# OpenImagingLab/AdaptiveISP

Hardware: AMD Instinct MI355X
Metric: ISP+YOLO forward images/sec @1280x720 bs8 (higher is better)
Workload: dtype bf16; 1 GPU; batch 8 x 1280x720 fp32 RGB, 5-step ISP schedule ['E', 'CCM', 'NLM', 'Shr', 'T'] (teacher-forced, policy/heads evaluated every step) + YOLOv3 forward @1280x736 bf16 (random-init weights); per_gpu_batch=8, global_batch=8, parallelism=replicas x1

## Files before the change

### adaptiveisp_amd/csrc/yolo_api.hip

```cpp
#include "yolo_internal.h"
#include <algorithm>
#include <atomic>
#include <cstdlib>
#include <cstring>
#include <mutex>
#include <unordered_map>
#include <vector>

using namespace adayolo;

static void magic_div(unsigned d, unsigned* magic, int* sh) {
    if (d <= 1) { *magic = 0; *sh = -1; return; }
    int L = 0;
    while ((1ull << L) < d) ++L;
    const unsigned long long num = 1ull << (31 + L);
    *magic = (unsigned)((num + d - 1) / d);
    *sh = L - 1;
}

static int code(hipError_t e, int on_invalid = ADAYOLO_ELAUNCH) {
    if (e == hipErrorInvalidValue) return on_invalid;
    return e == hipSuccess ? ADAYOLO_OK : ADAYOLO_ELAUNCH;
}

// ... 618 lines not shown
                       void* stream) {
    if (!in || !out || B <= 0 || H <= 0 || W <= 0 || C <= 0) return ADAYOLO_EINVAL;
    if (C % 8 || in_cstride % 8 || out_cstride % 8 || in_cstride < C || out_cstride < C) return ADAYOLO_ESHAPE;
    return code(launch_upsample2x(in, in_cstride, out, out_cstride, B, H, W, C, static_cast<hipStream_t>(stream)));
}

int adayolo_detect_decode(const void* raw, int raw_cstride, float* pred, int pred_rows, int row_offset,
                          const float* anchors_px, float det_stride, int B, int ny, int nx, int na, int no,
                          void* stream) {
    if (!raw || !pred || !anchors_px || B <= 0 || ny <= 0 || nx <= 0 || na <= 0 || no < 5) return ADAYOLO_EINVAL;
    if (raw_cstride < na * no || row_offset < 0 || row_offset + na * ny * nx > pred_rows) return ADAYOLO_ESHAPE;
    return code(launch_detect_decode(raw, raw_cstride, pred, pred_rows, row_offset, anchors_px, det_stride, B, ny, nx, na,
                                     no, static_cast<hipStream_t>(stream)));
}

size_t adayolo_nms_workspace_bytes(int n) {
    const size_t nb = (size_t)((n > 0 ? n : 0) + 63) / 64;
    return (size_t)(n > 0 ? n : 0) * nb * 8 + 8;
}

int adayolo_nms(const float* boxes_xyxy, int n, float iou_thres, int max_det, void* workspace, int32_t* keep,
                int32_t* num_keep, void* stream) {
    if (n < 0 || max_det <= 0 || !keep || !num_keep || (n > 0 && (!boxes_xyxy || !workspace))) return ADAYOLO_EINVAL;
    if (n > 30000 * 4) return ADAYOLO_ESHAPE;
    if (!(iou_thres >= 0.0f && iou_thres <= 1.0f)) return ADAYOLO_EINVAL;
    return code(launch_nms(boxes_xyxy, n, iou_thres, max_det, static_cast<unsigned long long*>(workspace), keep, num_keep,
                           static_cast<hipStream_t>(stream)));
}

static int detloss_check(const adayolo_loss_args* a, bool bwd) {
// ... 27 lines not shown
```

### adaptiveisp_amd/csrc/yolo_conv_pq.hip

```cpp
#include "yolo_device.h"
#include <type_traits>
#include <cstdlib>

namespace adayolo {
namespace pq {

template <int N> using IC = std::integral_constant<int, N>;

constexpr int BN = 128, BK = 32;
constexpr int kRow = BK * 2;
template <int MI> struct Geo {
    static constexpr int BM = 64 * MI;
    static constexpr int kATile = BM * kRow;
    static constexpr int kBuf = (BM + BN) * kRow;
    static constexpr int kRing = 3 * kBuf;
    static constexpr int kEpi = 4 * 32 * MI * kEpiPitch;
    static constexpr int kSmem = kRing > kEpi ? kRing : kEpi;
    static constexpr int NA = MI;
    static constexpr int NP = MI + 2;
};

__device__ __forceinline__ void fence() { __builtin_amdgcn_sched_barrier(0); }
#define PQ_SGB(mask, n) __builtin_amdgcn_sched_group_barrier(mask, n, 0)

template <int ABL, int MI>
__global__ __launch_bounds__(256, 2) void k_conv_pq(const ConvArgs a) {
    constexpr int BM = Geo<MI>::BM, kATile = Geo<MI>::kATile, kBuf = Geo<MI>::kBuf, NA = Geo<MI>::NA, NP = Geo<MI>::NP;
    constexpr int H1 = NP / 2;
    extern __shared__ __attribute__((aligned(16))) unsigned char smem[];
    const int tid = threadIdx.x, lane = tid & 63;
    const int wave = __builtin_amdgcn_readfirstlane(tid >> 6);
    const int wm = wave >> 1, wn = wave & 1;
    const int lid = xcd_remap(blockIdx.x, a.mtiles * a.ntiles);
    const int m0 = (lid / a.ntiles) * BM, n0 = (lid % a.ntiles) * BN;
    const int Kw = a.ks * a.ks * a.Cin;
    const int nK = Kw / BK;

    const unsigned guard = 2u * (unsigned)(a.W + 1) * (unsigned)a.in_cs;
    const __amdgpu_buffer_rsrc_t rsA =
        __builtin_amdgcn_make_buffer_rsrc((void*)((const unsigned char*)a.in - guard), 0, kRecords, kDescFlags);
// ... 189 lines not shown
#pragma unroll
                for (int it = 0; it < 4; ++it) {
                    r[it] = u32x4{0u, 0u, 0u, 0u};
                    if (ok[it]) r[it] = *reinterpret_cast<const u32x4*>(rp + (4 * mi + it) * rstep);
                }
            }
#pragma unroll
            for (int ni = 0; ni < 2; ++ni)
#pragma unroll
                for (int qd = 0; qd < 4; ++qd) {
                    f32x2 x0 = {acc[ni][mi][4 * qd], acc[ni][mi][4 * qd + 1]}, x1 = {acc[ni][mi][4 * qd + 2], acc[ni][mi][4 * qd + 3]};
                    if (kSilu) { x0 = silu_pk(x0); x1 = silu_pk(x1); }
                    *reinterpret_cast<u32x2*>(wr + mi * 32 * kEpiPitch + (ni * 32 + 8 * qd) * 2) =
                        u32x2{pack_bf16x2(x0.x, x0.y), pack_bf16x2(x1.x, x1.y)};
                }
            asm volatile("s_waitcnt lgkmcnt(0)" ::: "memory");
#pragma unroll
            for (int it = 0; it < 4; ++it) v[it] = *reinterpret_cast<const u32x4*>(rd + (mi * 32 + it * 8) * kEpiPitch);
            if (kKeep) {
#pragma unroll
                for (int it = 0; it < 4; ++it) {
                    if (ok[it]) *reinterpret_cast<u32x4*>(a.pre + (long)(mrow + 8 * (4 * mi + it)) * a.pre_cs + n) = v[it];
                    if (kAct) {
#pragma unroll
                        for (int j = 0; j < 4; ++j) v[it][j] = silu_bf16x2(v[it][j]);
                    }
                }
            }
            if (kRes) {
#pragma unroll
// ... 14 lines not shown
                }
                if (a.out) {
#pragma unroll
                    for (int it = 0; it < 4; ++it)
                        if (ok[it]) __builtin_nontemporal_store(v[it], reinterpret_cast<u32x4*>(op + (4 * mi + it) * ostep));
                }
#pragma unroll
                for (int it = 0; it < 4; ++it) {
#pragma unroll
                    for (int j = 0; j < 4; ++j) v[it][j] = dsilu_bf16x2(v[it][j], p[it][j]);
                    if (ok[it])
                        __builtin_nontemporal_store(v[it], reinterpret_cast<u32x4*>(a.gpre + (long)(mrow + 8 * (4 * mi + it)) * a.gpre_cs + n));
                }
                continue;
            }
#pragma unroll
            for (int it = 0; it < 4; ++it)
                if (ok[it]) __builtin_nontemporal_store(v[it], reinterpret_cast<u32x4*>(op + (4 * mi + it) * ostep));
        }
    };
    const std::false_type no{};
    const std::true_type yes{};
    if (a.gpre) {
        if (a.res) epilogue(no, yes, no, yes); else epilogue(no, no, no, yes);
    } else if (a.pre) {
        if (a.act == ADAYOLO_ACT_SILU) { if (a.res) epilogue(yes, yes, yes, no); else epilogue(yes, no, yes, no); }
        else { if (a.res) epilogue(no, yes, yes, no); else epilogue(no, no, yes, no); }
    } else if (a.act == ADAYOLO_ACT_SILU) {
        if (a.res) epilogue(yes, yes, no, no); else epilogue(yes, no, no, no);
    } else {
        if (a.res) epilogue(no, yes, no, no); else epilogue(no, no, no, no);
    }
}

template <int ABL, int MI = 4>
static hipError_t launch(ConvArgs a, hipStream_t s) {
    constexpr int kSmem = Geo<MI>::kSmem;
    static_assert(2 * kSmem <= 160 * 1024, "two workgroups per CU");
    a.mtiles = (a.M + Geo<MI>::BM - 1) / Geo<MI>::BM;
    auto kern = k_conv_pq<ABL, MI>;
    static bool configured = false;
    if (!configured) {
        hipError_t e = hipFuncSetAttribute(reinterpret_cast<const void*>(kern),
                                           hipFuncAttributeMaxDynamicSharedMemorySize, kSmem);
        if (e != hipSuccess) return e;
        configured = true;
    }
    int smem_bytes = kSmem;
#ifdef ADAYOLO_MEASURE
    static const int extra = getenv("ADAYOLO_PQ_EXTRA_SMEM") ? atoi(getenv("ADAYOLO_PQ_EXTRA_SMEM")) : 0;
    smem_bytes += extra;
    if (extra) (void)hipFuncSetAttribute(reinterpret_cast<const void*>(kern), hipFuncAttributeMaxDynamicSharedMemorySize, smem_bytes);
#endif
    hipLaunchKernelGGL(kern, dim3(a.mtiles * a.ntiles), dim3(256), smem_bytes, s, a);
    return hipGetLastError();
}

}

hipError_t launch_conv_pq(ConvArgs a, hipStream_t s, int variant) {
    const long nK = (long)a.ks * a.ks * a.Cin / 32;
    if (a.Cin % 32 || a.Cout % 128 || nK < 3 || a.sh_hw < 0 || a.sh_w < 0 || a.d2s_c) return hipErrorInvalidValue;
    const unsigned long long lim = 0xFFFFFF00ull - 64;
    const unsigned long long in_b = 2ull * a.B * a.H * a.W * a.in_cs + 4ull * (a.W + 1) * a.in_cs + 2ull * a.Cin;
    if (in_b > lim || 2ull * a.Cout * a.ks * a.ks * a.Cin > lim) return hipErrorInvalidValue;
    a.ntiles = a.Cout / pq::BN;
#ifdef ADAYOLO_MEASURE
    if (variant == 81) return pq::launch<1>(a, s);
    if (variant == 82) return pq::launch<2>(a, s);
    if (variant == 83) return pq::launch<3>(a, s);
#endif
    if (variant == 85) return pq::launch<0, 2>(a, s);
    return pq::launch<0>(a, s);
}

}
```

### adaptiveisp_amd/csrc/yolo_device.h

```cpp
#pragma once
#include "yolo_internal.h"

namespace adayolo {

typedef __attribute__((ext_vector_type(8))) __bf16 bf16x8;
typedef __attribute__((ext_vector_type(2))) __bf16 bf16x2;
typedef __attribute__((ext_vector_type(2))) float f32x2;
typedef __attribute__((ext_vector_type(4))) float f32x4;
typedef __attribute__((ext_vector_type(16))) float f32x16;
typedef __attribute__((ext_vector_type(2))) unsigned int u32x2;
typedef __attribute__((ext_vector_type(4))) unsigned int u32x4;
typedef __attribute__((ext_vector_type(4))) short s16x4;
typedef __attribute__((address_space(3))) void* lds_ptr_t;
typedef const __attribute__((address_space(1))) void* gbl_ptr_t;

__device__ __forceinline__ float bf16_to_f32(unsigned short h) { return __uint_as_float(((unsigned)h) << 16); }
__device__ __forceinline__ float lo_f(unsigned v) { return __uint_as_float(v << 16); }
__device__ __forceinline__ float hi_f(unsigned v) { return __uint_as_float(v & 0xFFFF0000u); }
__device__ __forceinline__ unsigned pack_bf16x2(float lo, float hi) {
    return __builtin_bit_cast(unsigned, __builtin_convertvector(f32x2{lo, hi}, bf16x2));
}
__device__ __forceinline__ unsigned short f32_to_bf16(float f) {
    unsigned u = __float_as_uint(f);
    u += 0x7FFFu + ((u >> 16) & 1u);
// ... 62 lines not shown
    return x * r;
}
__device__ __forceinline__ unsigned silu_bf16x2(unsigned v) {
    const f32x2 y = silu_pk(f32x2{__uint_as_float(v << 16), __uint_as_float(v & 0xFFFF0000u)});
    return __builtin_bit_cast(unsigned, __builtin_convertvector(y, bf16x2));
}
__device__ __forceinline__ float dsilu_f32(float g, float p) {
    const float s = __builtin_amdgcn_rcpf(1.0f + __builtin_amdgcn_exp2f(-1.44269504088896341f * p));
    return g * __builtin_fmaf(p * s, 1.0f - s, s);
}
__device__ __forceinline__ unsigned dsilu_bf16x2(unsigned g, unsigned p) {
    const f32x2 y = {dsilu_f32(__uint_as_float(g << 16), __uint_as_float(p << 16)),
                     dsilu_f32(__uint_as_float(g & 0xFFFF0000u), __uint_as_float(p & 0xFFFF0000u))};
    return __builtin_bit_cast(unsigned, __builtin_convertvector(y, bf16x2));
}
template <bool SILU>
__device__ __forceinline__ void bias_act_pack4(float a0, float a1, float a2, float a3, const float4 b, unsigned& lo, unsigned& hi) {
    f32x2 x0 = f32x2{a0, a1} + f32x2{b.x, b.y};
    f32x2 x1 = f32x2{a2, a3} + f32x2{b.z, b.w};
    if (SILU) { x0 = silu_pk(x0); x1 = silu_pk(x1); }
    lo = __builtin_bit_cast(unsigned, __builtin_convertvector(x0, bf16x2));
    hi = __builtin_bit_cast(unsigned, __builtin_convertvector(x1, bf16x2));
}

}
```

### adaptiveisp_amd/csrc/yolo_internal.h

```cpp
#pragma once
#include <hip/hip_runtime.h>
#include <stdint.h>
#include "../../include/adayolo.h"

namespace adayolo {

struct ConvArgs {
    const unsigned short* in; int in_cs;
    const unsigned short* w; const float* bias;
    const unsigned short* res; int res_cs;
    unsigned short* out; int out_cs;
    int B, H, W, Cin, Cout, Ho, Wo, ks, stride, pad, act;
    int M;
    int mtiles, ntiles;
    unsigned magic_hw, magic_w;
    int sh_hw, sh_w;
    const unsigned short* w2; const float* bias2;
    unsigned short* out2; int out2_cs;
    unsigned short* pre; int pre_cs;
    float* partial = nullptr; int* tickets = nullptr; int ksplit = 1;
    unsigned short* gpre = nullptr; int gpre_cs = 0;
    int d2s_c = 0;
    int chain_tile = 0;
};

struct ChainHead { int layer, lid, flag, pad; };
struct ChainDeps {
    int in_lo, in_n_need;
    int res_lo, res_n_need;
};
struct ChainArgs {
    unsigned char* ws;
    int* host_err;
    int off_layers, off_heads, off_deps, total, ndone;
    int stagger;
};
hipError_t launch_conv_chain(const ChainArgs& c, int grid, hipStream_t s);
enum ShapeFamily { kShapePp = 0, kShapePp128 = 1 };
int mfma_shape(ShapeFamily f);
hipError_t launch_conv_dma(ConvArgs a, hipStream_t s, int variant);
hipError_t launch_conv_dma2(ConvArgs a, hipStream_t s, int variant);
hipError_t launch_conv_small(ConvArgs a, hipStream_t s, int variant);
hipError_t launch_conv_pp(ConvArgs a, hipStream_t s, int variant);
hipError_t launch_conv_pp128(ConvArgs a, hipStream_t s, int variant);
size_t conv_pp128_splitk_bytes(const ConvArgs& a, int S);
hipError_t launch_conv_pp128_splitk(ConvArgs a, hipStream_t s, int S, void* workspace, size_t workspace_bytes);
hipError_t launch_bottleneck256(const void* x, int x_cs, const void* w1, const float* b1, const void* w2, const float* b2,
                                void* out, int out_cs, int B, int H, int W, hipStream_t s);
hipError_t launch_bottleneck_ws(const void* x, int x_cs, const void* w1, const float* b1, const void* w2, const float* b2,
                                void* out, int out_cs, int B, int H, int W, int C, hipStream_t s);
hipError_t launch_conv_k1(ConvArgs a, hipStream_t s);
hipError_t launch_conv_pq(ConvArgs a, hipStream_t s, int variant);
hipError_t launch_conv_ws(ConvArgs a, hipStream_t s, int variant);
hipError_t launch_stem(const float* img, const float* w, const float* bias, void* out, int out_cs, int B, int H,
                       int W, int Hp, int pad_top, float pad_value, int act, hipStream_t s, void* pre = nullptr, int pre_cs = 0);
hipError_t launch_letterbox_pack(const float* img, void* out, int out_cs, int B, int H, int W, int Hp, int pad_top,
                                 float pad_value, hipStream_t s);
hipError_t launch_stem_down(const float* img, const float* w0, const float* b0, const void* w1, const float* b1, void* out,
                            int out_cs, int B, int H, int W, int Hp, int pad_top, float pad_value, const void* w2,
                            const float* b2, void* out2, int out2_cs, hipStream_t s);
hipError_t launch_upsample2x(const void* in, int in_cs, void* out, int out_cs, int B, int H, int W, int C,
                             hipStream_t s);
hipError_t launch_detect_decode(const void* raw, int raw_cs, float* pred, int pred_rows, int row_offset,
                                const float* anchors_px, float det_stride, int B, int ny, int nx, int na, int no,
                                hipStream_t s);
hipError_t launch_silu_fwd(const void* pre, int pre_cs, const void* res, int res_cs, void* out, int out_cs, long npix,
                           int C, hipStream_t s);
// ... 15 lines not shown
```

### adaptiveisp_amd/csrc/yolo_misc.hip

```cpp
#include "yolo_device.h"

namespace adayolo {

constexpr int S_TW = 64, S_TH = 16, S_LW = S_TW + 2, S_LH = S_TH + 2;

__global__ __launch_bounds__(256) void k_stem(const float* __restrict__ img, const float* __restrict__ w,
                                              const float* __restrict__ bias, unsigned short* __restrict__ out,
                                              int out_cs, int H, int W, int Hp, int pad_top, float pad_value, int act,
                                              unsigned short* __restrict__ pre, int pre_cs) {
    __shared__ float tile[3 * S_LH * S_LW];
    const int tid = threadIdx.x, lane = tid & 63, wave = tid >> 6;
    const int b = blockIdx.z, x0 = blockIdx.x * S_TW, y0 = blockIdx.y * S_TH;
    const long plane = (long)H * W;
    const float* src = img + (long)b * 3 * plane;
    for (int i = tid; i < 3 * S_LH * S_LW; i += 256) {
        const int c = i / (S_LH * S_LW), r = i - c * (S_LH * S_LW);
        const int ly = r / S_LW, lx = r - ly * S_LW;
        const int gy = y0 - 1 + ly, gx = x0 - 1 + lx;
        float v = 0.0f;
        if (gy >= 0 && gy < Hp && gx >= 0 && gx < W) {
            const int sy = gy - pad_top;
            v = (sy >= 0 && sy < H) ? src[c * plane + (long)sy * W + gx] : pad_value;
        }
        tile[i] = v;
// ... 119 lines not shown
}

__global__ __launch_bounds__(256) void k_detect_decode(const unsigned short* __restrict__ raw, int raw_cs,
                                                       float* __restrict__ pred, int pred_rows, int row_offset,
                                                       const float* __restrict__ anchors_px, float det_stride, int ny,
                                                       int nx, int na, int no) {
    const int an = blockIdx.y;
    const long b = blockIdx.z;
    const int per_map = ny * nx * no;
    const float aw = anchors_px[2 * an], ah = anchors_px[2 * an + 1];
    const unsigned short* src = raw + b * ny * nx * raw_cs + an * no;
    float* dst = pred + (b * pred_rows + row_offset + (long)an * ny * nx) * no;
    for (int i = blockIdx.x * 256 + threadIdx.x; i < per_map; i += gridDim.x * 256) {
        const int cell = i / no, j = i - cell * no;
        const float t = bf16_to_f32(src[(long)cell * raw_cs + j]);
        const float s = __builtin_amdgcn_rcpf(1.0f + __builtin_amdgcn_exp2f(-1.44269504088896341f * t));
        float v = s;
        if (j < 4) {
            const int y = cell / nx, x = cell - y * nx;
            const float s2 = s * 2.0f;
            v = (j == 0) ? (s2 + ((float)x - 0.5f)) * det_stride
              : (j == 1) ? (s2 + ((float)y - 0.5f)) * det_stride
              : (j == 2) ? s2 * s2 * aw : s2 * s2 * ah;
        }
        dst[i] = v;
    }
}

constexpr int DC = 32;
__global__ __launch_bounds__(256) void k_detect_decode_tiled(const unsigned short* __restrict__ raw, int raw_cs,
                                                             float* __restrict__ pred, int pred_rows, int row_offset,
                                                             const float* __restrict__ anchors_px, float det_stride,
                                                             int ny, int nx, int na, int no) {
    extern __shared__ __attribute__((aligned(16))) unsigned char dsm[];
    unsigned short* l16 = reinterpret_cast<unsigned short*>(dsm);
    const int ncell = ny * nx;
    const int cell0 = blockIdx.x * DC;
    const int nc = min(DC, ncell - cell0);
// ... 24 lines not shown
                ++j;
                const int wr = j == no;
                j = wr ? 0 : j; an += wr;
            }
        }
    }
    __syncthreads();
    float* boxf = reinterpret_cast<float*>(dsm + (size_t)na * DC * no * 2);
    for (int idx = threadIdx.x; idx < na * nc; idx += 256) {
        const int an = (int)(((float)idx + 0.5f) / (float)nc), cl = idx - an * nc;
        const int cell = cell0 + cl;
        const int y = (int)(((float)cell + 0.5f) * inv_nx), x = cell - y * nx;
        const unsigned short* lp = l16 + (an * DC + cl) * no;
        float sg[4];
#pragma unroll
        for (int u = 0; u < 4; ++u) sg[u] = __builtin_amdgcn_rcpf(1.0f + __builtin_amdgcn_exp2f(-1.44269504088896341f * bf16_to_f32(lp[u])));
        float* bo = boxf + (an * DC + cl) * 4;
        bo[0] = (sg[0] * 2.0f + ((float)x - 0.5f)) * det_stride;
        bo[1] = (sg[1] * 2.0f + ((float)y - 0.5f)) * det_stride;
        bo[2] = (sg[2] * 2.0f) * (sg[2] * 2.0f) * anchors_px[2 * an];
        bo[3] = (sg[3] * 2.0f) * (sg[3] * 2.0f) * anchors_px[2 * an + 1];
    }
    __syncthreads();
    const int total = nc * no;
    for (int an = 0; an < na; ++an) {
        float* dst = pred + (b * pred_rows + row_offset + (long)an * ncell + cell0) * no;
        const unsigned char* la = dsm + (long)an * DC * no * 2;
        for (int e4 = threadIdx.x; 4 * e4 < total; e4 += 256) {
            const uint2 p = *reinterpret_cast<const uint2*>(la + 8 * e4);
            const float t[4] = {__uint_as_float(p.x << 16), __uint_as_float(p.x & 0xFFFF0000u),
                                __uint_as_float(p.y << 16), __uint_as_float(p.y & 0xFFFF0000u)};
            f32x4 o;
#pragma unroll
            for (int u = 0; u < 4; ++u) o[u] = __builtin_amdgcn_rcpf(1.0f + __builtin_amdgcn_exp2f(-1.44269504088896341f * t[u]));
            const int cl = (int)(((float)(4 * e4) + 0.5f) * inv_no), j0 = 4 * e4 - cl * no;
            if (j0 < 4 || j0 + 3 >= no) {
#pragma unroll
                for (int u = 0; u < 4; ++u) {
                    const int wrp = j0 + u >= no;
                    const int j = j0 + u - (wrp ? no : 0);
                    if (j < 4) o[u] = boxf[(an * DC + cl + wrp) * 4 + j];
                }
            }
            __builtin_nontemporal_store(o, reinterpret_cast<f32x4*>(dst + 4 * e4));
        }
    }
}

hipError_t launch_detect_decode(const void* raw, int raw_cs, float* pred, int pred_rows, int row_offset,
// ... 25 lines not shown
```

### adaptiveisp_amd/yolo/_lib.py

```python
import ctypes
import os

import torch

_HERE = os.path.dirname(os.path.dirname(os.path.abspath(__file__)))
LIB_PATH = os.environ.get("ADAYOLO_LIB") or os.path.join(_HERE, "csrc", "libadayolo.so")
ABI_VERSION = 9
ACT_NONE, ACT_SILU = 0, 1
EXPORTS = ("adayolo_conv_fwd", "adayolo_conv_fwd_variant", "adayolo_conv_fused1x1_fwd", "adayolo_conv1x1_stream_fwd", "adayolo_bottleneck256_fwd", "adayolo_bottleneck_ws_fwd", "adayolo_conv_keep_fwd", "adayolo_conv_splitk_fwd", "adayolo_conv_dsilu_fwd", "adayolo_conv_s2grad_fwd", "adayolo_conv_splitk_workspace_bytes", "adayolo_conv_chain_workspace_bytes", "adayolo_conv_chain_prepare", "adayolo_conv_chain_fwd", "adayolo_conv_chain_status", "adayolo_conv_chain_poll", "adayolo_conv_chain_tables", "adayolo_stem_fwd", "adayolo_upsample2x", "adayolo_detect_decode", "adayolo_nms", "adayolo_nms_workspace_bytes", "adayolo_stem_fwd_act", "adayolo_stem_keep_fwd", "adayolo_stem_down_fwd", "adayolo_letterbox_pack", "adayolo_silu_fwd", "adayolo_silu_bwd",
           "adayolo_zero_insert2x", "adayolo_upsample2x_bwd", "adayolo_image_grad", "adayolo_detloss_fwd", "adayolo_detloss_bwd",
           "adayolo_strerror", "adayolo_set_mfma_shape", "adayolo_get_mfma_shape",
           "adayolo_abi_version")
_lib = None


class AdayoloError(RuntimeError):
    pass


class LossLayer(ctypes.Structure):
    _fields_ = [("raw", ctypes.c_void_p), ("cs", ctypes.c_int), ("ny", ctypes.c_int), ("nx", ctypes.c_int),
                ("balance", ctypes.c_float), ("idx", ctypes.c_void_p), ("box", ctypes.c_void_p), ("n", ctypes.c_int),
                ("part", ctypes.c_void_p), ("tobj", ctypes.c_void_p), ("cnt", ctypes.c_void_p),
                ("grad", ctypes.c_void_p), ("grad_cs", ctypes.c_int)]
# ... 24 lines not shown
        raise AdayoloError(f"{LIB_PATH} not found: run __graft_entry__.build() (hipcc --offload-arch=gfx950); "
                           "the detector has no eager fallback")
    L = ctypes.CDLL(LIB_PATH)
    vp, ci, cf = ctypes.c_void_p, ctypes.c_int, ctypes.c_float
    L.adayolo_conv_fwd.argtypes = [vp, ci, vp, vp, vp, ci, vp, ci, ci, ci, ci, ci, ci, ci, ci, ci, vp]
    L.adayolo_conv_fwd_variant.argtypes = [vp, ci, vp, vp, vp, ci, vp, ci, ci, ci, ci, ci, ci, ci, ci, ci, ci, vp]
    L.adayolo_conv_fwd_variant.restype = ci
    L.adayolo_conv_fused1x1_fwd.argtypes = [vp, ci, vp, vp, vp, ci, vp, ci, ci, ci, ci, ci, ci, ci, ci, ci, vp, vp, vp, ci, ci, vp]
    L.adayolo_conv_fused1x1_fwd.restype = ci
    L.adayolo_bottleneck256_fwd.argtypes = [vp, ci, vp, vp, vp, vp, vp, ci, ci, ci, ci, vp]
    L.adayolo_bottleneck256_fwd.restype = ci
    L.adayolo_bottleneck_ws_fwd.argtypes = [vp, ci, vp, vp, vp, vp, vp, ci, ci, ci, ci, ci, vp]
    L.adayolo_bottleneck_ws_fwd.restype = ci
    L.adayolo_conv_keep_fwd.argtypes = [vp, ci, vp, vp, vp, ci, vp, ci, vp, ci, ci, ci, ci, ci, ci, ci, ci, ci, ci, vp]
    L.adayolo_conv_keep_fwd.restype = ci
    L.adayolo_stem_fwd.argtypes = [vp, vp, vp, vp, ci, ci, ci, ci, ci, ci, cf, ci, vp]
    L.adayolo_upsample2x.argtypes = [vp, ci, vp, ci, ci, ci, ci, ci, vp]
    L.adayolo_detect_decode.argtypes = [vp, ci, vp, ci, ci, vp, cf, ci, ci, ci, ci, ci, vp]
    cl = ctypes.c_long
    L.adayolo_stem_fwd_act.argtypes = [vp, vp, vp, vp, ci, ci, ci, ci, ci, ci, cf, ci, ci, vp]
    L.adayolo_stem_keep_fwd.argtypes = [vp, vp, vp, vp, ci, vp, ci, ci, ci, ci, ci, ci, cf, ci, vp]
    L.adayolo_stem_down_fwd.argtypes = [vp, vp, vp, vp, vp, vp, ci, ci, ci, ci, ci, ci, cf, vp, vp, vp, ci, vp]
    L.adayolo_stem_down_fwd.restype = ci
    L.adayolo_letterbox_pack.argtypes = [vp, vp, ci, ci, ci, ci, ci, ci, cf, vp]
    L.adayolo_letterbox_pack.restype = ci
    L.adayolo_silu_fwd.argtypes = [vp, ci, vp, ci, vp, ci, cl, ci, vp]
    L.adayolo_silu_bwd.argtypes = [vp, ci, vp, ci, vp, ci, vp, ci, ci, cl, ci, vp]
    L.adayolo_zero_insert2x.argtypes = [vp, ci, vp, ci, ci, ci, ci, ci, ci, ci, vp]
    L.adayolo_upsample2x_bwd.argtypes = [vp, ci, vp, ci, ci, ci, ci, ci, ci, vp]
    L.adayolo_image_grad.argtypes = [vp, ci, vp, ci, ci, ci, ci, ci, vp]
# ... 57 lines not shown
```

### adaptiveisp_amd/yolo/engine.py

```python
import collections
import ctypes
import os

import torch

from . import _lib
from .model import Bottleneck, Concat, Conv, Detect, DetectionModel

LETTERBOX_VALUE = 114.0 / 255.0


class _View:

    def __init__(self, buf, coff, C):
        self.buf, self.coff, self.C = buf, coff, C
        self.H, self.W, self.cs = buf.shape[1], buf.shape[2], buf.shape[3]

    @property
    def ptr(self):
        return self.buf.data_ptr() + 2 * self.coff

    def tensor(self):
        return self.buf[..., self.coff:self.coff + self.C]


def _pack_conv(w, b, pad_cout_to=None):
    w = w.detach().float().permute(0, 2, 3, 1).contiguous()
    b = b.detach().float().contiguous()
    if pad_cout_to is not None and w.shape[0] < pad_cout_to:
        extra = pad_cout_to - w.shape[0]
        w = torch.cat([w, w.new_zeros((extra,) + tuple(w.shape[1:]))], 0)
        b = torch.cat([b, b.new_zeros(extra)], 0)
    return w.to(torch.bfloat16).contiguous(), b


BNECK_WS_DEFAULT = "1"

ARG_RES, ARG_OUT, ARG_SHAPE, ARG_K, ARG_VARIANT = 4, 6, 8, 13, 16


class ConvShape(collections.namedtuple("ConvShape", "B H W cin cout k s act variant Ho Wo flops inp in_cs weight res res_cs "
                                                    "out out_cs")):
    __slots__ = ()

    @property
    def key(self):
        return tuple(self[:8])


def _conv_shape(args, kind="conv"):
# ... 338 lines not shown
            return 0

        def match(a, b, x, y):
            if (x.variant == 50 and x.cout == 256 and x.cin % 64 == 0 and
                    (y.cin, y.cout, y.k, y.s, y.act, y.res) == (256, 128, 1, 1, _lib.ACT_SILU, None) and
                    (y.inp, y.in_cs, y.B, y.H, y.W) == (x.out, x.out_cs, x.B, x.Ho, x.Wo)):
                w2p = self._weight(y).reshape(4, 32, 16, 2, 8).permute(0, 2, 3, 1, 4).contiguous()
                self._keep.append(w2p)
                return ("conv2", self.L.adayolo_conv_fused1x1_fwd,
                        list(a[:ARG_VARIANT]) + [ctypes.c_void_p(w2p.data_ptr()), b[3], b[6], b[7], 128])

        self.plan, n = _rewrite_pairs(self.plan, self.head_entries, match)
        self.fused_pairs += n
        self.fuse_chains()
        self.fuse_k1()
        return n

    def fuse_k1(self):
        self.k1_layers = getattr(self, "k1_layers", 0)
        if os.environ.get("ADAYOLO_K1", "0") != "1" or not self._pair_fusion:
            return 0
        n = 0
        for i, (kind, fn, a) in enumerate(self.plan):
            if i < self.head_entries or kind != "conv":
                continue
            x = _conv_shape(a)
            if not (x.k == 1 and x.s == 1 and x.res is None and x.cin in (256, 512) and x.cout % 256 == 0):
                continue
            w = self._weight(x)
            if w.shape[0] != x.cout or w.numel() != x.cout * x.cin:
# ... 186 lines not shown
                a[0] = ctypes.c_void_p(x.inp + c * Bc * x.H * x.W * x.in_cs * 2)
                a[ARG_OUT] = ctypes.c_void_p(x.out + c * Bc * x.Ho * x.Wo * x.out_cs * 2)
                a[ARG_SHAPE] = Bc
                rc = fn(*a, st)
                if rc != 0:
                    _lib.check(rc, "adayolo conv")
        for kind, fn, args in self.plan[(2 if nc > 1 else 1):]:
            rc = fn(*args, st)
            if rc != 0:
                _lib.check(rc, f"adayolo {kind}")
        return self.pred

    __call__ = forward

    def raw_maps(self):
        outs = []
        for v in self.raw:
            t = v.buf[..., : self.na * self.no].float()
            outs.append(t.view(self.B, v.H, v.W, self.na, self.no).permute(0, 3, 1, 2, 4).contiguous())
        return outs


def chain_runs(entries, cus, chain_min):
    out, i, n = [], 0, len(entries)
    while i < n:
        j = i
        while j < n and entries[j][0] and entries[j][1] > cus:
            j += 1
        if i < j < n and entries[j][0]:
            j += 1
# ... 9 lines not shown
```

### include/adayolo.h

```cpp
#ifndef ADAYOLO_H_
#define ADAYOLO_H_

#include <stddef.h>
#include <stdint.h>

#ifdef __cplusplus
extern "C" {
#endif

#define ADAYOLO_ABI_VERSION 9

#define ADAYOLO_ACT_NONE 0
#define ADAYOLO_ACT_SILU 1

#define ADAYOLO_OK       0
#define ADAYOLO_EINVAL  -1
#define ADAYOLO_ESHAPE  -2
#define ADAYOLO_ELAUNCH -3

#define ADAYOLO_MFMA_SHAPE_PP_DEFAULT    16
#define ADAYOLO_MFMA_SHAPE_PP128_DEFAULT 16
int adayolo_set_mfma_shape(int family, int shape);
int adayolo_get_mfma_shape(int family);

int adayolo_conv_fwd(const void* in, int in_cstride,
// ... 93 lines not shown
                     int gp_cstride, void* grad_res, int gr_cstride, int accumulate_res, long npix, int C, void* stream);
int adayolo_zero_insert2x(const void* in, int in_cstride, void* out, int out_cstride, int B, int Ho, int Wo, int H, int W,
                          int C, void* stream);
int adayolo_upsample2x_bwd(const void* grad_out, int go_cstride, void* grad_in, int gi_cstride, int accumulate, int B,
                           int H, int W, int C, void* stream);
int adayolo_image_grad(const void* grad_nhwc, int g_cstride, float* grad_img, int B, int H, int W, int Hp, int pad_top,
                       void* stream);

int adayolo_upsample2x(const void* in, int in_cstride, void* out, int out_cstride,
                       int B, int H, int W, int C, void* stream);

int adayolo_detect_decode(const void* raw, int raw_cstride, float* pred, int pred_rows, int row_offset,
                          const float* anchors_px, float det_stride,
                          int B, int ny, int nx, int na, int no, void* stream);

size_t adayolo_nms_workspace_bytes(int n);
int adayolo_nms(const float* boxes_xyxy, int n, float iou_thres, int max_det, void* workspace,
                int32_t* keep, int32_t* num_keep, void* stream);

typedef struct adayolo_loss_layer {
    const void* raw; int cs; int ny, nx; float balance;
    const int32_t* idx; const float* box; int n;
    float* part; float* tobj; float* cnt;
    void* grad; int grad_cs;
} adayolo_loss_layer;
typedef struct adayolo_loss_args {
    adayolo_loss_layer layer[4];
    int nl, B, na, nc, no;
    float hyp_box, hyp_obj, hyp_cls, cp, cn, cls_pw, obj_pw;
    float* loss;
// ... 14 lines not shown
```

Measured before the change: 1999 images/sec.

## Fuse 1x1 conv epilogue with detect decode and 2x nearest upsample

```diff
diff --git a/adaptiveisp_amd/csrc/yolo_api.hip b/adaptiveisp_amd/csrc/yolo_api.hip
--- a/adaptiveisp_amd/csrc/yolo_api.hip
+++ b/adaptiveisp_amd/csrc/yolo_api.hip
@@ -656,6 +656,32 @@
                                      no, static_cast<hipStream_t>(stream)));
 }
 
+int adayolo_conv1x1_decode_fwd(const void* in, int in_cstride, const void* weight, const float* bias, int B, int H, int W, int Cin,
+                               int Cout, int variant, float* pred, int pred_rows, int row_offset, const float* anchors_px,
+                               float det_stride, int na, int no, void* stream) {
+    if (!in || !weight || !bias || !pred || !anchors_px) return ADAYOLO_EINVAL;
+    if (B <= 0 || H <= 0 || W <= 0 || Cin <= 0 || Cout <= 0 || na <= 0 || no < 5) return ADAYOLO_EINVAL;
+    if (family_of(variant) != kPq) return ADAYOLO_EINVAL;
+    if (Cin % 8 || Cout % 8 || in_cstride % 8 || in_cstride < Cin) return ADAYOLO_ESHAPE;
+    if (Cout < na * no || row_offset < 0 || row_offset + (long)na * H * W > pred_rows) return ADAYOLO_ESHAPE;
+    ConvArgs a;
+    const int rc = conv_fill(a, in, in_cstride, weight, bias, nullptr, 0, nullptr, 0, B, H, W, Cin, Cout, 1, 1, 0, ADAYOLO_ACT_NONE);
+    if (rc != ADAYOLO_OK) return rc;
+    a.pred = pred; a.pred_rows = pred_rows; a.row_offset = row_offset;
+    a.anchors_px = anchors_px; a.det_stride = det_stride; a.na = na; a.no = no;
+    return code(launch_conv_pq_decode(a, static_cast<hipStream_t>(stream), variant), ADAYOLO_ESHAPE);
+}
+
+int adayolo_conv1x1_up2_fwd(const void* in, int in_cstride, const void* weight, const float* bias, void* out, int out_cstride,
+                            int B, int H, int W, int Cin, int Cout, int act, int variant, void* stream) {
+    ConvArgs a;
+    const int rc = conv_args(a, in, in_cstride, weight, bias, nullptr, 0, out, out_cstride, B, H, W, Cin, Cout, 1, 1, act);
+    if (rc != ADAYOLO_OK) return rc;
+    if (family_of(variant) != kPq) return ADAYOLO_EINVAL;
+    if (4L * a.M > 0x7fffffffL) return ADAYOLO_ESHAPE;
+    return code(launch_conv_pq_up2(a, static_cast<hipStream_t>(stream), variant), ADAYOLO_ESHAPE);
+}
+
 size_t adayolo_nms_workspace_bytes(int n) {
     const size_t nb = (size_t)((n > 0 ? n : 0) + 63) / 64;
     return (size_t)(n > 0 ? n : 0) * nb * 8 + 8;
diff --git a/adaptiveisp_amd/csrc/yolo_conv_pq.hip b/adaptiveisp_amd/csrc/yolo_conv_pq.hip
--- a/adaptiveisp_amd/csrc/yolo_conv_pq.hip
+++ b/adaptiveisp_amd/csrc/yolo_conv_pq.hip
@@ -23,7 +23,11 @@
 __device__ __forceinline__ void fence() { __builtin_amdgcn_sched_barrier(0); }
 #define PQ_SGB(mask, n) __builtin_amdgcn_sched_group_barrier(mask, n, 0)
 
-template <int ABL, int MI>
+__device__ __forceinline__ int div_magic(int n, unsigned magic, int sh) { return (int)(__umulhi((unsigned)n, magic) >> sh); }
+
+enum Tail { kTailNone = 0, kTailDecode = 1, kTailUp2 = 2 };
+
+template <int ABL, int MI, int TAIL = kTailNone>
 __global__ __launch_bounds__(256, 2) void k_conv_pq(const ConvArgs a) {
     constexpr int BM = Geo<MI>::BM, kATile = Geo<MI>::kATile, kBuf = Geo<MI>::kBuf, NA = Geo<MI>::NA, NP = Geo<MI>::NP;
     constexpr int H1 = NP / 2;
@@ -243,6 +247,7 @@
                     *reinterpret_cast<u32x2*>(wr + mi * 32 * kEpiPitch + (ni * 32 + 8 * qd) * 2) =
                         u32x2{pack_bf16x2(x0.x, x0.y), pack_bf16x2(x1.x, x1.y)};
                 }
+            if constexpr (TAIL == kTailDecode) continue;
             asm volatile("s_waitcnt lgkmcnt(0)" ::: "memory");
 #pragma unroll
             for (int it = 0; it < 4; ++it) v[it] = *reinterpret_cast<const u32x4*>(rd + (mi * 32 + it * 8) * kEpiPitch);
@@ -287,6 +292,22 @@
                 }
                 continue;
             }
+            if constexpr (TAIL == kTailUp2) {
+#pragma unroll
+                for (int it = 0; it < 4; ++it) {
+                    if (!ok[it]) continue;
+                    const int m = mrow + 8 * (4 * mi + it);
+                    const int b = div_magic(m, a.magic_hw, a.sh_hw);
+                    const int rem = m - b * (a.Ho * a.Wo);
+                    const int y = div_magic(rem, a.magic_w, a.sh_w), x = rem - y * a.Wo;
+                    unsigned short* const o = a.out + (((long)b * 2 * a.Ho + 2 * y) * (2L * a.Wo) + 2 * x) * a.out_cs + n;
+                    *reinterpret_cast<u32x4*>(o) = v[it];
+                    *reinterpret_cast<u32x4*>(o + a.out_cs) = v[it];
+                    *reinterpret_cast<u32x4*>(o + 2L * a.Wo * a.out_cs) = v[it];
+                    *reinterpret_cast<u32x4*>(o + (2L * a.Wo + 1) * a.out_cs) = v[it];
+                }
+                continue;
+            }
 #pragma unroll
             for (int it = 0; it < 4; ++it)
                 if (ok[it]) __builtin_nontemporal_store(v[it], reinterpret_cast<u32x4*>(op + (4 * mi + it) * ostep));
@@ -294,7 +315,67 @@
     };
     const std::false_type no{};
     const std::true_type yes{};
-    if (a.gpre) {
+    if constexpr (TAIL == kTailUp2) {
+        if (a.act == ADAYOLO_ACT_SILU) epilogue(yes, no, no, no); else epilogue(no, no, no, no);
+    } else if constexpr (TAIL == kTailDecode) {
+        epilogue(no, no, no, no);
+        barrier_lgkm();
+        constexpr int kRegion = 32 * MI * kEpiPitch;
+        const int ncell = a.Ho * a.Wo, used = a.na * a.no;
+        const int mend = m0 + BM < a.M ? m0 + BM : a.M;
+        const float inv_no = 1.0f / (float)a.no;
+        int b = div_magic(m0, a.magic_hw, a.sh_hw);
+        for (int ms = m0; ms < mend; ++b) {
+            const int c0 = ms - b * ncell;
+            const int nc = (mend - ms < ncell - c0) ? mend - ms : ncell - c0;
+            const int total = nc * a.no;
+            for (int an = 0; an < a.na; ++an) {
+                const int jlo = n0 - an * a.no > 0 ? n0 - an * a.no : 0;
+                int jhi = (n0 + BN < used ? n0 + BN : used) - an * a.no;
+                jhi = jhi < a.no ? jhi : a.no;
+                if (jlo >= jhi) continue;
+                const long e0 = (((long)b * a.pred_rows + a.row_offset + (long)an * ncell + c0)) * a.no;
+                float* const dst = a.pred + e0;
+                const int mis = (int)(e0 & 3);
+                const float aw = a.anchors_px[2 * an], ah = a.anchors_px[2 * an + 1];
+                const int cbase = an * a.no - n0;
+                for (int e = 4 * tid - mis; e < total; e += 4 * 256) {
+                    const int ef = e < 0 ? 0 : e;
+                    int cl = (int)(((float)ef + 0.5f) * inv_no), j = ef - cl * a.no;
+                    f32x4 o;
+                    unsigned own = 0u;
+#pragma unroll
+                    for (int u = 0; u < 4; ++u) {
+                        o[u] = 0.0f;
+                        if (e + u < 0 || e + u >= total) continue;
+                        if (j >= jlo && j < jhi) {
+                            const int p = ms - m0 + cl, c = cbase + j;
+                            const int pw = p / (32 * MI);
+                            const unsigned short t = *reinterpret_cast<const unsigned short*>(
+                                smem + (2 * pw + (c >> 6)) * kRegion + (p - pw * (32 * MI)) * kEpiPitch + (c & 63) * 2);
+                            float s = detect_sigmoid(bf16_to_f32(t));
+                            if (j < 4) {
+                                const int cell = c0 + cl;
+                                const int y = div_magic(cell, a.magic_w, a.sh_w), x = cell - y * a.Wo;
+                                s = detect_box(j, s, x, y, a.det_stride, aw, ah);
+                            }
+                            o[u] = s;
+                            own |= 1u << u;
+                        }
+                        if (++j == a.no) { j = 0; ++cl; }
+                    }
+                    if (own == 15u) {
+                        __builtin_nontemporal_store(o, reinterpret_cast<f32x4*>(dst + e));
+                    } else {
+#pragma unroll
+                        for (int u = 0; u < 4; ++u)
+                            if (own & (1u << u)) dst[e + u] = o[u];
+                    }
+                }
+            }
+            ms += nc;
+        }
+    } else if (a.gpre) {
         if (a.res) epilogue(no, yes, no, yes); else epilogue(no, no, no, yes);
     } else if (a.pre) {
         if (a.act == ADAYOLO_ACT_SILU) { if (a.res) epilogue(yes, yes, yes, no); else epilogue(yes, no, yes, no); }
@@ -306,12 +387,12 @@
     }
 }
 
-template <int ABL, int MI = 4>
+template <int ABL, int MI = 4, int TAIL = kTailNone>
 static hipError_t launch(ConvArgs a, hipStream_t s) {
     constexpr int kSmem = Geo<MI>::kSmem;
     static_assert(2 * kSmem <= 160 * 1024, "two workgroups per CU");
     a.mtiles = (a.M + Geo<MI>::BM - 1) / Geo<MI>::BM;
-    auto kern = k_conv_pq<ABL, MI>;
+    auto kern = k_conv_pq<ABL, MI, TAIL>;
     static bool configured = false;
     if (!configured) {
         hipError_t e = hipFuncSetAttribute(reinterpret_cast<const void*>(kern),
@@ -331,12 +412,37 @@
 
 }
 
-hipError_t launch_conv_pq(ConvArgs a, hipStream_t s, int variant) {
+static bool pq_serves(const ConvArgs& a) {
     const long nK = (long)a.ks * a.ks * a.Cin / 32;
-    if (a.Cin % 32 || a.Cout % 128 || nK < 3 || a.sh_hw < 0 || a.sh_w < 0 || a.d2s_c) return hipErrorInvalidValue;
+    if (a.Cin % 32 || a.Cout % 128 || nK < 3 || a.sh_hw < 0 || a.sh_w < 0 || a.d2s_c) return false;
     const unsigned long long lim = 0xFFFFFF00ull - 64;
     const unsigned long long in_b = 2ull * a.B * a.H * a.W * a.in_cs + 4ull * (a.W + 1) * a.in_cs + 2ull * a.Cin;
-    if (in_b > lim || 2ull * a.Cout * a.ks * a.ks * a.Cin > lim) return hipErrorInvalidValue;
+    return in_b <= lim && 2ull * a.Cout * a.ks * a.ks * a.Cin <= lim;
+}
+static bool pq_tail_ok(const ConvArgs& a, int variant) {
+    return pq_serves(a) && (variant == 80 || variant == 85) && a.ks == 1 && a.stride == 1 && !a.res && !a.pre && !a.gpre && !a.w2;
+}
+
+hipError_t launch_conv_pq_decode(ConvArgs a, hipStream_t s, int variant) {
+    if (!pq_tail_ok(a, variant) || a.act != ADAYOLO_ACT_NONE) return hipErrorInvalidValue;
+    const long level = (long)a.na * a.Ho * a.Wo;
+    if (a.na < 1 || a.no < 5 || a.no > 255 || a.na * a.no > a.Cout || a.row_offset < 0 || a.row_offset + level > a.pred_rows ||
+        (reinterpret_cast<uintptr_t>(a.pred) & 15) != 0)
+        return hipErrorInvalidValue;
+    a.ntiles = a.Cout / pq::BN;
+    if (variant == 85) return pq::launch<0, 2, pq::kTailDecode>(a, s);
+    return pq::launch<0, 4, pq::kTailDecode>(a, s);
+}
+
+hipError_t launch_conv_pq_up2(ConvArgs a, hipStream_t s, int variant) {
+    if (!pq_tail_ok(a, variant) || a.out_cs % 8 || (reinterpret_cast<uintptr_t>(a.out) & 15) != 0) return hipErrorInvalidValue;
+    a.ntiles = a.Cout / pq::BN;
+    if (variant == 85) return pq::launch<0, 2, pq::kTailUp2>(a, s);
+    return pq::launch<0, 4, pq::kTailUp2>(a, s);
+}
+
+hipError_t launch_conv_pq(ConvArgs a, hipStream_t s, int variant) {
+    if (!pq_serves(a)) return hipErrorInvalidValue;
     a.ntiles = a.Cout / pq::BN;
 #ifdef ADAYOLO_MEASURE
     if (variant == 81) return pq::launch<1>(a, s);
diff --git a/adaptiveisp_amd/csrc/yolo_device.h b/adaptiveisp_amd/csrc/yolo_device.h
--- a/adaptiveisp_amd/csrc/yolo_device.h
+++ b/adaptiveisp_amd/csrc/yolo_device.h
@@ -100,6 +100,16 @@
                      dsilu_f32(__uint_as_float(g & 0xFFFF0000u), __uint_as_float(p & 0xFFFF0000u))};
     return __builtin_bit_cast(unsigned, __builtin_convertvector(y, bf16x2));
 }
+__device__ __forceinline__ float detect_sigmoid(float t) {
+    return __builtin_amdgcn_rcpf(1.0f + __builtin_amdgcn_exp2f(-1.44269504088896341f * t));
+}
+__device__ __forceinline__ float detect_box(int j, float s, int x, int y, float det_stride, float aw, float ah) {
+    const float s2 = s * 2.0f;
+    return j == 0 ? (s2 + ((float)x - 0.5f)) * det_stride
+         : j == 1 ? (s2 + ((float)y - 0.5f)) * det_stride
+         : j == 2 ? s2 * s2 * aw : s2 * s2 * ah;
+}
+
 template <bool SILU>
 __device__ __forceinline__ void bias_act_pack4(float a0, float a1, float a2, float a3, const float4 b, unsigned& lo, unsigned& hi) {
     f32x2 x0 = f32x2{a0, a1} + f32x2{b.x, b.y};
diff --git a/adaptiveisp_amd/csrc/yolo_internal.h b/adaptiveisp_amd/csrc/yolo_internal.h
--- a/adaptiveisp_amd/csrc/yolo_internal.h
+++ b/adaptiveisp_amd/csrc/yolo_internal.h
@@ -22,6 +22,8 @@
     unsigned short* gpre = nullptr; int gpre_cs = 0;
     int d2s_c = 0;
     int chain_tile = 0;
+    float* pred = nullptr; const float* anchors_px = nullptr; float det_stride = 0.0f;
+    int pred_rows = 0, row_offset = 0, na = 0, no = 0;
 };
 
 struct ChainHead { int layer, lid, flag, pad; };
@@ -51,6 +53,8 @@
                                 void* out, int out_cs, int B, int H, int W, int C, hipStream_t s);
 hipError_t launch_conv_k1(ConvArgs a, hipStream_t s);
 hipError_t launch_conv_pq(ConvArgs a, hipStream_t s, int variant);
+hipError_t launch_conv_pq_decode(ConvArgs a, hipStream_t s, int variant);
+hipError_t launch_conv_pq_up2(ConvArgs a, hipStream_t s, int variant);
 hipError_t launch_conv_ws(ConvArgs a, hipStream_t s, int variant);
 hipError_t launch_stem(const float* img, const float* w, const float* bias, void* out, int out_cs, int B, int H,
                        int W, int Hp, int pad_top, float pad_value, int act, hipStream_t s, void* pre = nullptr, int pre_cs = 0);
diff --git a/adaptiveisp_amd/csrc/yolo_misc.hip b/adaptiveisp_amd/csrc/yolo_misc.hip
--- a/adaptiveisp_amd/csrc/yolo_misc.hip
+++ b/adaptiveisp_amd/csrc/yolo_misc.hip
@@ -157,14 +157,11 @@
     for (int i = blockIdx.x * 256 + threadIdx.x; i < per_map; i += gridDim.x * 256) {
         const int cell = i / no, j = i - cell * no;
         const float t = bf16_to_f32(src[(long)cell * raw_cs + j]);
-        const float s = __builtin_amdgcn_rcpf(1.0f + __builtin_amdgcn_exp2f(-1.44269504088896341f * t));
+        const float s = detect_sigmoid(t);
         float v = s;
         if (j < 4) {
             const int y = cell / nx, x = cell - y * nx;
-            const float s2 = s * 2.0f;
-            v = (j == 0) ? (s2 + ((float)x - 0.5f)) * det_stride
-              : (j == 1) ? (s2 + ((float)y - 0.5f)) * det_stride
-              : (j == 2) ? s2 * s2 * aw : s2 * s2 * ah;
+            v = detect_box(j, s, x, y, det_stride, aw, ah);
         }
         dst[i] = v;
     }
@@ -219,12 +216,11 @@
         const unsigned short* lp = l16 + (an * DC + cl) * no;
         float sg[4];
 #pragma unroll
-        for (int u = 0; u < 4; ++u) sg[u] = __builtin_amdgcn_rcpf(1.0f + __builtin_amdgcn_exp2f(-1.44269504088896341f * bf16_to_f32(lp[u])));
+        for (int u = 0; u < 4; ++u) sg[u] = detect_sigmoid(bf16_to_f32(lp[u]));
         float* bo = boxf + (an * DC + cl) * 4;
-        bo[0] = (sg[0] * 2.0f + ((float)x - 0.5f)) * det_stride;
-        bo[1] = (sg[1] * 2.0f + ((float)y - 0.5f)) * det_stride;
-        bo[2] = (sg[2] * 2.0f) * (sg[2] * 2.0f) * anchors_px[2 * an];
-        bo[3] = (sg[3] * 2.0f) * (sg[3] * 2.0f) * anchors_px[2 * an + 1];
+        const float aw = anchors_px[2 * an], ah = anchors_px[2 * an + 1];
+#pragma unroll
+        for (int u = 0; u < 4; ++u) bo[u] = detect_box(u, sg[u], x, y, det_stride, aw, ah);
     }
     __syncthreads();
     const int total = nc * no;
@@ -237,7 +233,7 @@
                                 __uint_as_float(p.y << 16), __uint_as_float(p.y & 0xFFFF0000u)};
             f32x4 o;
 #pragma unroll
-            for (int u = 0; u < 4; ++u) o[u] = __builtin_amdgcn_rcpf(1.0f + __builtin_amdgcn_exp2f(-1.44269504088896341f * t[u]));
+            for (int u = 0; u < 4; ++u) o[u] = detect_sigmoid(t[u]);
             const int cl = (int)(((float)(4 * e4) + 0.5f) * inv_no), j0 = 4 * e4 - cl * no;
             if (j0 < 4 || j0 + 3 >= no) {
 #pragma unroll
diff --git a/adaptiveisp_amd/yolo/_lib.py b/adaptiveisp_amd/yolo/_lib.py
--- a/adaptiveisp_amd/yolo/_lib.py
+++ b/adaptiveisp_amd/yolo/_lib.py
@@ -5,9 +5,9 @@
 
 _HERE = os.path.dirname(os.path.dirname(os.path.abspath(__file__)))
 LIB_PATH = os.environ.get("ADAYOLO_LIB") or os.path.join(_HERE, "csrc", "libadayolo.so")
-ABI_VERSION = 9
+ABI_VERSION = 10
 ACT_NONE, ACT_SILU = 0, 1
-EXPORTS = ("adayolo_conv_fwd", "adayolo_conv_fwd_variant", "adayolo_conv_fused1x1_fwd", "adayolo_conv1x1_stream_fwd", "adayolo_bottleneck256_fwd", "adayolo_bottleneck_ws_fwd", "adayolo_conv_keep_fwd", "adayolo_conv_splitk_fwd", "adayolo_conv_dsilu_fwd", "adayolo_conv_s2grad_fwd", "adayolo_conv_splitk_workspace_bytes", "adayolo_conv_chain_workspace_bytes", "adayolo_conv_chain_prepare", "adayolo_conv_chain_fwd", "adayolo_conv_chain_status", "adayolo_conv_chain_poll", "adayolo_conv_chain_tables", "adayolo_stem_fwd", "adayolo_upsample2x", "adayolo_detect_decode", "adayolo_nms", "adayolo_nms_workspace_bytes", "adayolo_stem_fwd_act", "adayolo_stem_keep_fwd", "adayolo_stem_down_fwd", "adayolo_letterbox_pack", "adayolo_silu_fwd", "adayolo_silu_bwd",
+EXPORTS = ("adayolo_conv_fwd", "adayolo_conv_fwd_variant", "adayolo_conv_fused1x1_fwd", "adayolo_conv1x1_stream_fwd", "adayolo_bottleneck256_fwd", "adayolo_bottleneck_ws_fwd", "adayolo_conv_keep_fwd", "adayolo_conv1x1_decode_fwd", "adayolo_conv1x1_up2_fwd", "adayolo_conv_splitk_fwd", "adayolo_conv_dsilu_fwd", "adayolo_conv_s2grad_fwd", "adayolo_conv_splitk_workspace_bytes", "adayolo_conv_chain_workspace_bytes", "adayolo_conv_chain_prepare", "adayolo_conv_chain_fwd", "adayolo_conv_chain_status", "adayolo_conv_chain_poll", "adayolo_conv_chain_tables", "adayolo_stem_fwd", "adayolo_upsample2x", "adayolo_detect_decode", "adayolo_nms", "adayolo_nms_workspace_bytes", "adayolo_stem_fwd_act", "adayolo_stem_keep_fwd", "adayolo_stem_down_fwd", "adayolo_letterbox_pack", "adayolo_silu_fwd", "adayolo_silu_bwd",
            "adayolo_zero_insert2x", "adayolo_upsample2x_bwd", "adayolo_image_grad", "adayolo_detloss_fwd", "adayolo_detloss_bwd",
            "adayolo_strerror", "adayolo_set_mfma_shape", "adayolo_get_mfma_shape",
            "adayolo_abi_version")
@@ -62,6 +62,10 @@
     L.adayolo_bottleneck_ws_fwd.restype = ci
     L.adayolo_conv_keep_fwd.argtypes = [vp, ci, vp, vp, vp, ci, vp, ci, vp, ci, ci, ci, ci, ci, ci, ci, ci, ci, ci, vp]
     L.adayolo_conv_keep_fwd.restype = ci
+    L.adayolo_conv1x1_decode_fwd.argtypes = [vp, ci, vp, vp, ci, ci, ci, ci, ci, ci, vp, ci, ci, vp, cf, ci, ci, vp]
+    L.adayolo_conv1x1_decode_fwd.restype = ci
+    L.adayolo_conv1x1_up2_fwd.argtypes = [vp, ci, vp, vp, vp, ci, ci, ci, ci, ci, ci, ci, ci, vp]
+    L.adayolo_conv1x1_up2_fwd.restype = ci
     L.adayolo_stem_fwd.argtypes = [vp, vp, vp, vp, ci, ci, ci, ci, ci, ci, cf, ci, vp]
     L.adayolo_upsample2x.argtypes = [vp, ci, vp, ci, ci, ci, ci, ci, vp]
     L.adayolo_detect_decode.argtypes = [vp, ci, vp, ci, ci, vp, cf, ci, ci, ci, ci, ci, vp]
diff --git a/adaptiveisp_amd/yolo/engine.py b/adaptiveisp_amd/yolo/engine.py
--- a/adaptiveisp_amd/yolo/engine.py
+++ b/adaptiveisp_amd/yolo/engine.py
@@ -34,6 +34,7 @@
     return w.to(torch.bfloat16).contiguous(), b
 
 
+FUSE_TAIL_DEFAULT = "up"
 BNECK_WS_DEFAULT = "1"
 
 ARG_RES, ARG_OUT, ARG_SHAPE, ARG_K, ARG_VARIANT = 4, 6, 8, 13, 16
@@ -402,6 +403,57 @@
         self.fused_pairs += n
         self.fuse_chains()
         self.fuse_k1()
+        self.fuse_tail()
+        return n
+
+    ESHAPE = -2
+
+    def _sole_reader(self, x, reader_ops):
+        dst = next((o["dst"] for o in self.ops if o["kind"] == "conv" and o["dst"].ptr == x.out), None)
+        if dst is None or dst.coff != 0 or dst.cs != x.cout:
+            return False
+        base = dst.buf.data_ptr()
+        return sum(1 for o in self.ops for k in ("src", "res") if o.get(k) is not None and o[k].buf.data_ptr() == base) == reader_ops
+
+    def fuse_tail(self):
+        self.fused_tail = getattr(self, "fused_tail", 0)
+        mode = os.environ.get("ADAYOLO_FUSE_TAIL", FUSE_TAIL_DEFAULT)
+        if not self._pair_fusion or mode not in ("1", "up", "decode"):
+            return 0
+        kinds = ("decode", "up") if mode == "1" else (mode,)
+        P, out, i, n = self.plan, [], 0, 0
+        with torch.cuda.device(self.dev):
+            st = _lib.stream_ptr()
+            while i < len(P):
+                e = None
+                if i >= self.head_entries and i + 1 < len(P) and P[i][0] == "conv" and P[i + 1][0] in kinds:
+                    a, (kind, _, t) = P[i][2], P[i + 1]
+                    x = _conv_shape(a)
+                    if (x.variant in (80, 85) and (x.k, x.s, x.res) == (1, 1, None) and
+                            (t[0].value, t[1]) == (x.out, x.out_cs)):
+                        if kind == "decode" and x.act == _lib.ACT_NONE and tuple(t[7:10]) == (x.B, x.H, x.W) and \
+                                self._sole_reader(x, 0):
+                            e = ("convdec", self.L.adayolo_conv1x1_decode_fwd,
+                                 [a[0], a[1], a[2], a[3], x.B, x.H, x.W, x.cin, x.cout, x.variant, *t[2:7], *t[10:12]])
+                        elif kind == "up" and tuple(t[4:8]) == (x.B, x.H, x.W, x.cout) and self._sole_reader(x, 1):
+                            e = ("convup", self.L.adayolo_conv1x1_up2_fwd,
+                                 [a[0], a[1], a[2], a[3], t[2], t[3], x.B, x.H, x.W, x.cin, x.cout, x.act, x.variant])
+                    if e is not None:
+                        rc = e[1](*e[2], st)
+                        if rc == self.ESHAPE:
+                            e = None
+                        else:
+                            _lib.check(rc, f"adayolo {e[0]}")
+                if e is not None:
+                    if e[0] == "convdec":
+                        self._raw_convs = getattr(self, "_raw_convs", []) + [P[i]]
+                    out.append(e)
+                    i, n = i + 2, n + 1
+                else:
+                    out.append(P[i])
+                    i += 1
+        self.plan = out
+        self.fused_tail += n
         return n
 
     def fuse_k1(self):
@@ -618,6 +670,8 @@
     __call__ = forward
 
     def raw_maps(self):
+        for kind, fn, args in getattr(self, "_raw_convs", []):
+            _lib.check(fn(*args, _lib.stream_ptr()), f"adayolo {kind}")
         outs = []
         for v in self.raw:
             t = v.buf[..., : self.na * self.no].float()
diff --git a/include/adayolo.h b/include/adayolo.h
--- a/include/adayolo.h
+++ b/include/adayolo.h
@@ -8,7 +8,7 @@
 extern "C" {
 #endif
 
-#define ADAYOLO_ABI_VERSION 9
+#define ADAYOLO_ABI_VERSION 10
 
 #define ADAYOLO_ACT_NONE 0
 #define ADAYOLO_ACT_SILU 1
@@ -132,6 +132,13 @@
                           const float* anchors_px, float det_stride,
                           int B, int ny, int nx, int na, int no, void* stream);
 
+int adayolo_conv1x1_decode_fwd(const void* in, int in_cstride, const void* weight, const float* bias, int B, int H, int W, int Cin,
+                               int Cout, int variant, float* pred, int pred_rows, int row_offset, const float* anchors_px,
+                               float det_stride, int na, int no, void* stream);
+
+int adayolo_conv1x1_up2_fwd(const void* in, int in_cstride, const void* weight, const float* bias, void* out, int out_cstride,
+                            int B, int H, int W, int Cin, int Cout, int act, int variant, void* stream);
+
 size_t adayolo_nms_workspace_bytes(int n);
 int adayolo_nms(const float* boxes_xyxy, int n, float iou_thres, int max_det, void* workspace,
                 int32_t* keep, int32_t* num_keep, void* stream);
```

Result: no change. 1999 images/sec (median of 2 runs) (+0.0%).
